# adr-arroyo/PointCloudComparator

Hardware: AMD Instinct MI355X
Metric: nn_queries_per_sec (higher is better)
Workload: dtype f32; 1 GPU; C3: 10M x 10M XYZRGB (32-B stride), k=1 NN; step = index build over 10000000 references + 10000000 queries on each GPU (10000000 over 1 GPU); backend=none, engine=grid, references=10000000, queries_per_gpu=10000000, queries_total=10000000, point_stride_bytes=32

## Files before the change

### pointcloudcomparator_amd/csrc/cellsort_mp.hip

```cpp
#include "pcc_internal.hpp"
#include "grid_device.hpp"
#include "lane_ops.hpp"
#include <algorithm>

namespace pcc {

constexpr int MP_T = 256;
constexpr unsigned int MP_F2 = 2048;
constexpr unsigned int MP_B2 = 128;
constexpr unsigned int MP_MAX_B1 = 256;
constexpr unsigned int MP_MAX_G = 512;
constexpr unsigned int MP_SLICE2 = 8192;
constexpr unsigned int MP_STAGE_BYTES = 32768;
constexpr unsigned int MP_WIN = 8;
#ifndef PCC_MP_STAGE_PTS
#define PCC_MP_STAGE_PTS 3072
#endif
#ifndef PCC_MP_STAGE_ORD
#define PCC_MP_STAGE_ORD 6144
#endif
constexpr unsigned int MP_FINE_STAGE_PTS = PCC_MP_STAGE_PTS, MP_FINE_STAGE_ORD = PCC_MP_STAGE_ORD;

struct MpPlan {
    unsigned int F1, F2, B1, G1, slice1;
};
static MpPlan mp_plan(unsigned int ncells_cap, unsigned int n) {
    MpPlan p;
    p.F2 = MP_F2;
    while ((unsigned long long)p.F2 * MP_B2 * MP_MAX_B1 < (unsigned long long)ncells_cap + 1) p.F2 *= 2;
    p.F1 = p.F2 * MP_B2;
    p.B1 = (ncells_cap + p.F1) / p.F1;
    p.G1 = (n + 16383) / 16384;
    if (p.G1 > MP_MAX_G) p.G1 = MP_MAX_G;
    if (p.G1 < 1) p.G1 = 1;
    p.slice1 = (n + p.G1 - 1) / p.G1;
    return p;
}

__device__ __forceinline__ unsigned int mp_cell(const float4& v, const GridParams& g, bool voxel) {
    return voxel ? voxel_id(v, g) : cell_id(v, g);
}
__device__ __forceinline__ unsigned int mp_cell(const uint2& v, const GridParams&, bool) { return v.x; }
__device__ __forceinline__ unsigned int mp_position(const float4& v) { return (unsigned int)__float_as_int(v.w); }
__device__ __forceinline__ unsigned int mp_position(const uint2& v) { return v.y; }
template <class E> __device__ __forceinline__ E mp_make(const float4& v, unsigned int cell, unsigned int pos);
template <> __device__ __forceinline__ float4 mp_make<float4>(const float4& v, unsigned int, unsigned int) { return v; }
template <> __device__ __forceinline__ uint2 mp_make<uint2>(const float4&, unsigned int cell, unsigned int pos) { return make_uint2(cell, pos); }

__global__ void __launch_bounds__(MP_T)
k_mp_hist1(const float4* __restrict__ pts, unsigned int n, const GridDev* __restrict__ gd, unsigned int F1, unsigned int B1,
           unsigned int slice, unsigned int* __restrict__ H, unsigned int* __restrict__ zero, unsigned int n_zero) {
    for (unsigned int z = blockIdx.x * MP_T + threadIdx.x; z < n_zero; z += gridDim.x * MP_T) zero[z] = 0u;
    __shared__ unsigned int cnt[MP_MAX_B1];
    const GridParams g = gd->g;
    const bool voxel = gd->voxel != 0;
    for (unsigned int b = threadIdx.x; b < B1; b += MP_T) cnt[b] = 0;
    __syncthreads();
    const unsigned int beg = blockIdx.x * slice, end = min(n, beg + slice);
    for (unsigned int i0 = beg + threadIdx.x; i0 < end; i0 += 4 * MP_T) {
        float4 v[4];
#pragma unroll
        for (int u = 0; u < 4; ++u)
            if (i0 + u * MP_T < end) v[u] = pts[i0 + u * MP_T];
#pragma unroll
        for (int u = 0; u < 4; ++u)
            if (i0 + u * MP_T < end && __float_as_int(v[u].w) >= 0) atomicAdd(&cnt[mp_cell(v[u], g, voxel) / F1], 1u);
    }
    __syncthreads();
    for (unsigned int b = threadIdx.x; b < B1; b += MP_T) H[(size_t)b * gridDim.x + blockIdx.x] = cnt[b];
    if (blockIdx.x == 0 && threadIdx.x == 0) H[(size_t)B1 * gridDim.x] = 0;
}

template <class E>
__global__ void __launch_bounds__(MP_T)
k_mp_scatter1(const float4* __restrict__ pts, unsigned int n, const GridDev* __restrict__ gd, unsigned int F1, unsigned int B1,
              unsigned int slice, const unsigned int* __restrict__ H, E* __restrict__ out) {
    __shared__ unsigned int cur[MP_MAX_B1];
    const GridParams g = gd->g;
    const bool voxel = gd->voxel != 0;
    for (unsigned int b = threadIdx.x; b < B1; b += MP_T) cur[b] = H[(size_t)b * gridDim.x + blockIdx.x];
    __syncthreads();
    const unsigned int beg = blockIdx.x * slice, end = min(n, beg + slice);
    for (unsigned int i0 = beg + threadIdx.x; i0 < end; i0 += 4 * MP_T) {
        float4 v[4];
#pragma unroll
        for (int u = 0; u < 4; ++u)
            if (i0 + u * MP_T < end) v[u] = pts[i0 + u * MP_T];
#pragma unroll
        for (int u = 0; u < 4; ++u)
            if (i0 + u * MP_T < end && __float_as_int(v[u].w) >= 0) {
                const unsigned int c = mp_cell(v[u], g, voxel);
                out[atomicAdd(&cur[c / F1], 1u)] = mp_make<E>(v[u], c, i0 + u * MP_T);
            }
    }
}

__global__ void __launch_bounds__(MP_T)
k_mp_hist1_cells(const unsigned int* __restrict__ cells, unsigned int n, unsigned int F1, unsigned int B1, unsigned int slice,
                 unsigned int* __restrict__ H, unsigned int* __restrict__ zero, unsigned int n_zero) {
    for (unsigned int z = blockIdx.x * MP_T + threadIdx.x; z < n_zero; z += gridDim.x * MP_T) zero[z] = 0u;
    __shared__ unsigned int cnt[MP_MAX_B1];
    for (unsigned int b = threadIdx.x; b < B1; b += MP_T) cnt[b] = 0;
    __syncthreads();
    const unsigned int beg = blockIdx.x * slice, end = min(n, beg + slice);
    for (unsigned int i0 = beg + threadIdx.x; i0 < end; i0 += 8 * MP_T) {
        unsigned int c[8];
#pragma unroll
        for (int u = 0; u < 8; ++u) c[u] = i0 + u * MP_T < end ? cells[i0 + u * MP_T] : 0xffffffffu;
#pragma unroll
        for (int u = 0; u < 8; ++u)
            if (c[u] != 0xffffffffu) atomicAdd(&cnt[c[u] / F1], 1u);
    }
    __syncthreads();
    for (unsigned int b = threadIdx.x; b < B1; b += MP_T) H[(size_t)b * gridDim.x + blockIdx.x] = cnt[b];
    if (blockIdx.x == 0 && threadIdx.x == 0) H[(size_t)B1 * gridDim.x] = 0;
}
__global__ void __launch_bounds__(MP_T)
k_mp_scatter1_cells(const unsigned int* __restrict__ cells, unsigned int n, unsigned int F1, unsigned int B1, unsigned int slice,
                    const unsigned int* __restrict__ H, uint2* __restrict__ out) {
    __shared__ unsigned int cur[MP_MAX_B1];
    for (unsigned int b = threadIdx.x; b < B1; b += MP_T) cur[b] = H[(size_t)b * gridDim.x + blockIdx.x];
    __syncthreads();
    const unsigned int beg = blockIdx.x * slice, end = min(n, beg + slice);
    for (unsigned int i0 = beg + threadIdx.x; i0 < end; i0 += 8 * MP_T) {
        unsigned int c[8];
#pragma unroll
        for (int u = 0; u < 8; ++u) c[u] = i0 + u * MP_T < end ? cells[i0 + u * MP_T] : 0xffffffffu;
#pragma unroll
        for (int u = 0; u < 8; ++u)
            if (c[u] != 0xffffffffu) out[atomicAdd(&cur[c[u] / F1], 1u)] = make_uint2(c[u], i0 + u * MP_T);
    }
}

constexpr unsigned int MP_TILE1 = 2048;
template <class E>
__global__ void __launch_bounds__(MP_T)
k_mp_scatter1_staged(const float4* __restrict__ pts, unsigned int n, const GridDev* __restrict__ gd, unsigned int F1, unsigned int B1,
                     unsigned int slice, const unsigned int* __restrict__ H, E* __restrict__ out) {
    constexpr int PER = MP_TILE1 / MP_T;
    __shared__ unsigned int cur[MP_MAX_B1], tcnt[MP_MAX_B1], tstart[MP_MAX_B1];
    __shared__ unsigned short sb[MP_TILE1];
    __shared__ __attribute__((aligned(16))) unsigned char stage_raw[MP_TILE1 * sizeof(E)];
    E* stage = reinterpret_cast<E*>(stage_raw);
    const GridParams g = gd->g;
    const bool voxel = gd->voxel != 0;
    for (unsigned int b = threadIdx.x; b < B1; b += MP_T) cur[b] = H[(size_t)b * gridDim.x + blockIdx.x];
    const unsigned int beg = blockIdx.x * slice, end = min(n, beg + slice);
    for (unsigned int t0 = beg; t0 < end; t0 += MP_TILE1) {
        for (unsigned int b = threadIdx.x; b < MP_MAX_B1; b += MP_T) tcnt[b] = 0;
        __syncthreads();
        float4 v[PER];
        unsigned int bk[PER], rk[PER];
#pragma unroll
        for (int u = 0; u < PER; ++u) {
            const unsigned int i = t0 + threadIdx.x + u * MP_T;
            v[u] = make_float4(0.f, 0.f, 0.f, __int_as_float(-1));
            if (i < end) v[u] = pts[i];
        }
#pragma unroll
        for (int u = 0; u < PER; ++u) {
            bk[u] = 0xffffffffu;
            rk[u] = 0;
            if (__float_as_int(v[u].w) >= 0) {
                bk[u] = mp_cell(v[u], g, voxel);
                rk[u] = atomicAdd(&tcnt[bk[u] / F1], 1u);
            }
        }
        __syncthreads();
        if (threadIdx.x < 64) {
            unsigned int c[4], sum = 0;
#pragma unroll
            for (int j = 0; j < 4; ++j) { c[j] = tcnt[4 * threadIdx.x + j]; sum += c[j]; }
            unsigned int ex = wave_incl_scan_add(sum) - sum;
#pragma unroll
            for (int j = 0; j < 4; ++j) { tstart[4 * threadIdx.x + j] = ex; ex += c[j]; }
        }
        __syncthreads();
#pragma unroll
        for (int u = 0; u < PER; ++u)
            if (bk[u] != 0xffffffffu) {
                const unsigned int b = bk[u] / F1, slot = tstart[b] + rk[u];
                stage[slot] = mp_make<E>(v[u], bk[u], t0 + threadIdx.x + u * MP_T);
                sb[slot] = (unsigned short)b;
            }
        __syncthreads();
        const unsigned int tile_n = tstart[MP_MAX_B1 - 1] + tcnt[MP_MAX_B1 - 1];
        for (unsigned int j = threadIdx.x; j < tile_n; j += MP_T) {
            const unsigned int b = sb[j];
            out[cur[b] + (j - tstart[b])] = stage[j];
        }
        __syncthreads();
        for (unsigned int b = threadIdx.x; b < MP_MAX_B1; b += MP_T) cur[b] += tcnt[b];
    }
}

__device__ __forceinline__ unsigned int mp_pair(unsigned int c, unsigned int F1, unsigned int F2) {
    return (c / F1) * MP_B2 + (c % F1) / F2;
}

template <bool PLACE, class E>
__global__ void __launch_bounds__(MP_T)
k_mp_level2(const E* __restrict__ in, const unsigned int* __restrict__ n_valid_ptr, const GridDev* __restrict__ gd,
            unsigned int F1, unsigned int F2, unsigned int* __restrict__ C, E* __restrict__ out) {
    constexpr unsigned int SLICE = PLACE ? MP_STAGE_BYTES / sizeof(E) : MP_SLICE2;
    __shared__ unsigned int cnt[MP_WIN * MP_B2];
    __shared__ __attribute__((aligned(16))) unsigned char stage_raw[PLACE ? MP_STAGE_BYTES : 16];
    E* stage = reinterpret_cast<E*>(stage_raw);
    const GridParams g = gd->g;
    const bool voxel = gd->voxel != 0;
    const unsigned int n = *n_valid_ptr;
    const unsigned int beg = blockIdx.x * SLICE, end = min(n, beg + SLICE);
    if (beg >= end) return;
    const unsigned int w0 = (mp_cell(in[beg], g, voxel) / F1) * MP_B2;
    for (unsigned int k = threadIdx.x; k < MP_WIN * MP_B2; k += MP_T) cnt[k] = 0;
    __syncthreads();
    for (unsigned int i0 = beg + threadIdx.x; i0 < end; i0 += 4 * MP_T) {
        E v[4];
#pragma unroll
        for (int u = 0; u < 4; ++u)
            if (i0 + u * MP_T < end) v[u] = in[i0 + u * MP_T];
#pragma unroll
        for (int u = 0; u < 4; ++u) {
            if (i0 + u * MP_T >= end) break;
            if (PLACE) stage[i0 + u * MP_T - beg] = v[u];
            const unsigned int pr = mp_pair(mp_cell(v[u], g, voxel), F1, F2);
            if (pr - w0 < MP_WIN * MP_B2) atomicAdd(&cnt[pr - w0], 1u);
            else if (!PLACE) atomicAdd(&C[pr], 1u);
            else out[atomicAdd(&C[pr], 1u)] = v[u];
        }
    }
    __syncthreads();
    for (unsigned int k = threadIdx.x; k < MP_WIN * MP_B2; k += MP_T) {
        const unsigned int c = cnt[k];
        if (c) {
            if (!PLACE) atomicAdd(&C[w0 + k], c);
            else cnt[k] = atomicAdd(&C[w0 + k], c);
        }
    }
    if (!PLACE) return;
    __syncthreads();
    for (unsigned int j = threadIdx.x; j < end - beg; j += MP_T) {
        const E v = stage[j];
        const unsigned int pr = mp_pair(mp_cell(v, g, voxel), F1, F2);
        if (pr - w0 < MP_WIN * MP_B2) out[atomicAdd(&cnt[pr - w0], 1u)] = v;
    }
}

__device__ __forceinline__ void mp_store_point(float4* out, unsigned int pos, const float4& v) { if (out) out[pos] = v; }
__device__ __forceinline__ void mp_store_point(float4*, unsigned int, const uint2&) {}

template <bool REFS, class E>
__device__ __forceinline__ void mp_fine_block(unsigned int* lds, const E* __restrict__ in, unsigned int beg, unsigned int end, unsigned int cell0,
                                              const GridParams& g, bool voxel, unsigned int F2, float4* __restrict__ out_pts,
                                              unsigned int* __restrict__ out_order, unsigned int* __restrict__ cell_start) {
    unsigned int* cnt = lds;
    unsigned int* wsum = lds + F2;
    const unsigned int ncells = (unsigned int)g.ncells;
    for (unsigned int f = threadIdx.x; f < F2; f += MP_T) cnt[f] = 0;
    __syncthreads();
    for (unsigned int j0 = beg + threadIdx.x; j0 < end; j0 += 4 * MP_T) {
        E v[4];
#pragma unroll
        for (int u = 0; u < 4; ++u)
            if (j0 + u * MP_T < end) v[u] = in[j0 + u * MP_T];
#pragma unroll
        for (int u = 0; u < 4; ++u)
            if (j0 + u * MP_T < end) atomicAdd(&cnt[mp_cell(v[u], g, voxel) - cell0], 1u);
    }
    __syncthreads();
    const unsigned int per = (F2 + MP_T - 1) / MP_T;
    const unsigned int f0 = threadIdx.x * per, f1 = min(F2, f0 + per);
    unsigned int s = 0;
    for (unsigned int f = f0; f < f1; ++f) s += cnt[f];
    const unsigned int lane = threadIdx.x & 63, wave = threadIdx.x >> 6;
    const unsigned int inc = wave_incl_scan_add(s);
    if (lane == 63) wsum[wave] = inc;
    __syncthreads();
    unsigned int run = beg + inc - s;
    for (unsigned int w = 0; w < wave; ++w) run += wsum[w];
    for (unsigned int f = f0; f < f1; ++f) {
        const unsigned int c = cnt[f];
        cnt[f] = run;
        if (REFS && cell0 + f <= ncells) cell_start[cell0 + f] = run;
        run += c;
    }
    __syncthreads();
    const unsigned int stage_cap = out_pts ? MP_FINE_STAGE_PTS : MP_FINE_STAGE_ORD;
    const bool staged = end - beg <= stage_cap;
    float4* st_pts = reinterpret_cast<float4*>(lds + ((F2 + 4 + 3) & ~3u));
    unsigned int* st_ord = reinterpret_cast<unsigned int*>(st_pts + (out_pts ? MP_FINE_STAGE_PTS : 0));
    for (unsigned int j0 = beg + threadIdx.x; j0 < end; j0 += 4 * MP_T) {
        E v[4];
#pragma unroll
        for (int u = 0; u < 4; ++u)
            if (j0 + u * MP_T < end) v[u] = in[j0 + u * MP_T];
#pragma unroll
        for (int u = 0; u < 4; ++u) {
            if (j0 + u * MP_T >= end) break;
            const unsigned int pos = atomicAdd(&cnt[mp_cell(v[u], g, voxel) - cell0], 1u);
            if (staged) {
                mp_store_point(out_pts ? st_pts : nullptr, pos - beg, v[u]);
                if (out_order) st_ord[pos - beg] = mp_position(v[u]);
            } else {
                mp_store_point(out_pts, pos, v[u]);
                if (out_order) out_order[pos] = mp_position(v[u]);
            }
        }
    }
    if (staged) {
        __syncthreads();
        for (unsigned int i = threadIdx.x; i < end - beg; i += MP_T) {
            if (out_pts) out_pts[beg + i] = st_pts[i];
            if (out_order) out_order[beg + i] = st_ord[i];
        }
    }
}

#ifndef PCC_MP_LIGHT_PTS
#define PCC_MP_LIGHT_PTS 1024
#endif
#ifndef PCC_MP_LIGHT_ORD
#define PCC_MP_LIGHT_ORD 1024
#endif
template <class E> struct MpWave;
template <> struct MpWave<float4> {
    typedef float4 Staged;
    static constexpr unsigned int LIGHT = PCC_MP_LIGHT_PTS;
    static __device__ __forceinline__ float4 staged(const float4& v) { return v; }
    static __device__ __forceinline__ void store(float4* out_pts, unsigned int*, unsigned int pos, const float4& v) { out_pts[pos] = v; }
};
template <> struct MpWave<uint2> {
    typedef unsigned int Staged;
    static constexpr unsigned int LIGHT = PCC_MP_LIGHT_ORD;
    static __device__ __forceinline__ unsigned int staged(const uint2& v) { return v.y; }
    static __device__ __forceinline__ void store(float4*, unsigned int* out_order, unsigned int pos, unsigned int v) { out_order[pos] = v; }
};
template <class E> constexpr unsigned int mp_wave_words() {
    return MP_F2 / 2 + MpWave<E>::LIGHT * (unsigned int)(sizeof(typename MpWave<E>::Staged) / sizeof(unsigned int));
}
static_assert(PCC_MP_LIGHT_PTS % 64 == 0 && PCC_MP_LIGHT_ORD % 64 == 0 && PCC_MP_LIGHT_PTS < 65536 && PCC_MP_LIGHT_ORD < 65536,
              "a light bucket is whole rounds of a wave and fits a 16-bit counter");

template <bool REFS, class E>
__device__ __forceinline__ void mp_fine_wave(unsigned int* cnt , const E* __restrict__ in, unsigned int beg, unsigned int n,
                                             unsigned int cell0, const GridParams& g, bool voxel, float4* __restrict__ out_pts,
                                             unsigned int* __restrict__ out_order, unsigned int* __restrict__ cell_start) {
    typedef MpWave<E> W;
    constexpr unsigned int PER = W::LIGHT / 64;
    const unsigned int ncells = (unsigned int)g.ncells;
    const unsigned int lane = threadIdx.x & 63;
    if (n == 0) {
        for (unsigned int f = lane; f < MP_F2; f += 64)
            if (cell0 + f <= ncells) cell_start[cell0 + f] = beg;
        return;
    }
    unsigned short* cnt16 = reinterpret_cast<unsigned short*>(cnt);
    typename W::Staged* stage = reinterpret_cast<typename W::Staged*>(cnt + MP_F2 / 2);
    E v[PER];
#pragma unroll
    for (unsigned int u = 0; u < PER; ++u) v[u] = in[beg + min(lane + 64 * u, n - 1)];
    for (unsigned int k = lane; k < MP_F2 / 8; k += 64) reinterpret_cast<uint4*>(cnt)[k] = make_uint4(0u, 0u, 0u, 0u);
    wave_lds_sync();
    unsigned int key[PER];
#pragma unroll
    for (unsigned int u = 0; u < PER; ++u)
        if (lane + 64 * u < n) {
            const unsigned int c = (mp_cell(v[u], g, voxel) - cell0) & (MP_F2 - 1), sh = 16 * (c & 1);
            const unsigned int old = atomicAdd(&cnt[c >> 1], 1u << sh);
            key[u] = c | ((old >> sh) & 0xffffu) << 16;
        }
    wave_lds_sync();
    unsigned int base = 0;
#pragma unroll 8
    for (unsigned int step = 0; step < MP_F2 / 64; ++step) {
        const unsigned int f = 64 * step + lane;
        const unsigned int c = cnt16[f];
        const unsigned int inc = wave_incl_scan_add(c);
        const unsigned int first = base + inc - c;
        cnt16[f] = (unsigned short)first;
        if (REFS && cell0 + f <= ncells) cell_start[cell0 + f] = beg + first;
        base += __builtin_amdgcn_readlane(inc, 63);
    }
    wave_lds_sync();
#pragma unroll
    for (unsigned int u = 0; u < PER; ++u)
        if (lane + 64 * u < n) key[u] = cnt16[key[u] & 0xffffu] + (key[u] >> 16);
#pragma unroll
    for (unsigned int u = 0; u < PER; ++u)
        if (lane + 64 * u < n) stage[key[u]] = W::staged(v[u]);
    wave_lds_sync();
    for (unsigned int i = lane; i < n; i += 64) W::store(out_pts, out_order, beg + i, stage[i]);
}

template <class E> constexpr unsigned int mp_once_cap() { return MP_T * MpWave<E>::LIGHT / 64; }
template <class E> constexpr unsigned int mp_once_words() {
    return MP_F2 + 4 + mp_once_cap<E>() * (unsigned int)(sizeof(typename MpWave<E>::Staged) / sizeof(unsigned int));
}
template <bool REFS, class E>
__device__ __forceinline__ void mp_fine_once(unsigned int* lds, const E* __restrict__ in, unsigned int beg, unsigned int n, unsigned int cell0,
                                             const GridParams& g, bool voxel, float4* __restrict__ out_pts,
                                             unsigned int* __restrict__ out_order, unsigned int* __restrict__ cell_start) {
    typedef MpWave<E> W;
    constexpr unsigned int PER = W::LIGHT / 64;
    unsigned int* cnt = lds;
    unsigned int* wsum = lds + MP_F2;
    typename W::Staged* stage = reinterpret_cast<typename W::Staged*>(lds + MP_F2 + 4);
    const unsigned int ncells = (unsigned int)g.ncells;
    E v[PER];
#pragma unroll
    for (unsigned int u = 0; u < PER; ++u) v[u] = in[beg + min(threadIdx.x + MP_T * u, n - 1)];
    for (unsigned int f = threadIdx.x; f < MP_F2; f += MP_T) cnt[f] = 0;
    __syncthreads();
    unsigned int key[PER];
#pragma unroll
    for (unsigned int u = 0; u < PER; ++u)
        if (threadIdx.x + MP_T * u < n) {
            const unsigned int c = (mp_cell(v[u], g, voxel) - cell0) & (MP_F2 - 1);
            key[u] = c | atomicAdd(&cnt[c], 1u) << 16;
        }
    __syncthreads();
    constexpr unsigned int per = MP_F2 / MP_T;
    const unsigned int f0 = threadIdx.x * per;
    unsigned int s = 0;
#pragma unroll
    for (unsigned int f = f0; f < f0 + per; ++f) s += cnt[f];
    const unsigned int lane = threadIdx.x & 63, wave = threadIdx.x >> 6;
    const unsigned int inc = wave_incl_scan_add(s);
    if (lane == 63) wsum[wave] = inc;
    __syncthreads();
    unsigned int run = inc - s;
    for (unsigned int w = 0; w < wave; ++w) run += wsum[w];
#pragma unroll
    for (unsigned int f = f0; f < f0 + per; ++f) {
        const unsigned int c = cnt[f];
        cnt[f] = run;
        if (REFS && cell0 + f <= ncells) cell_start[cell0 + f] = beg + run;
        run += c;
    }
    __syncthreads();
#pragma unroll
    for (unsigned int u = 0; u < PER; ++u)
        if (threadIdx.x + MP_T * u < n) key[u] = cnt[key[u] & 0xffffu] + (key[u] >> 16);
#pragma unroll
    for (unsigned int u = 0; u < PER; ++u)
        if (threadIdx.x + MP_T * u < n) stage[key[u]] = W::staged(v[u]);
    __syncthreads();
    for (unsigned int i = threadIdx.x; i < n; i += MP_T) W::store(out_pts, out_order, beg + i, stage[i]);
}
static_assert(MP_T * PCC_MP_LIGHT_PTS / 64 < 65536 && MP_T * PCC_MP_LIGHT_ORD / 64 < 65536, "a rank of the one-read block form fits 16 bits");

template <bool REFS, class E>
__global__ void __launch_bounds__(MP_T)
k_mp_fine(const E* __restrict__ in, const unsigned int* __restrict__ ends , const GridDev* __restrict__ gd,
          unsigned int F2, unsigned int n_block, unsigned int light, float4* __restrict__ out_pts, unsigned int* __restrict__ out_order,
          unsigned int* __restrict__ cell_start) {
    extern __shared__ __attribute__((aligned(16))) unsigned int lds[];
    const GridParams g = gd->g;
    const bool voxel = gd->voxel != 0;
    const unsigned int ncells = (unsigned int)g.ncells;
    const bool block = blockIdx.x < n_block;
    const unsigned int wave = __builtin_amdgcn_readfirstlane(threadIdx.x >> 6);
    const unsigned int b = block ? blockIdx.x : 4 * (blockIdx.x - n_block) + wave;
    const unsigned int cell0 = b * F2;
    if (cell0 > ncells) return;
    const unsigned int beg = b ? ends[b - 1] : 0u, end = ends[b];
    if (!REFS && beg == end) return;
    if (block) {
        if (light == 0 || end - beg > mp_once_cap<E>()) mp_fine_block<REFS, E>(lds, in, beg, end, cell0, g, voxel, F2, out_pts, out_order, cell_start);
        else if (end - beg > light) mp_fine_once<REFS, E>(lds, in, beg, end - beg, cell0, g, voxel, out_pts, out_order, cell_start);
    } else if (end - beg <= light) {
        mp_fine_wave<REFS, E>(lds + wave * mp_wave_words<E>(), in, beg, end - beg, cell0, g, voxel, out_pts, out_order, cell_start);
    }
}

int cell_sort_mp(pcc_index* ix, const float4* pts, size_t n_pts, bool refs, float4* out_pts, unsigned int* out_order,
                 unsigned int* cell_start, unsigned int** n_sorted_dev, const GridDev* gd_override,
                 unsigned int nc_cap_override) {
    hipStream_t s = ix->stream;
    const unsigned int n = (unsigned int)n_pts;
    const unsigned int ncap = gd_override ? nc_cap_override : ix->nc_cap;
    const MpPlan p = mp_plan(ncap, n);
    const GridDev* gd = gd_override ? gd_override : ix->d_grid.as<GridDev>();
    const unsigned int np = p.B1 * MP_B2;
    PCC_TRY(ix->mp_a.reserve((size_t)n * sizeof(float4) + 256));
    PCC_TRY(ix->mp_b.reserve((size_t)n * sizeof(float4) + 256));
    const size_t h_elems = (size_t)p.B1 * p.G1 + 1;
    PCC_TRY(ix->scratch_b.reserve(((h_elems + 3) & ~(size_t)3) * sizeof(unsigned int)));
    PCC_TRY(ix->mp_c.reserve(((size_t)np + 8) * sizeof(unsigned int)));
    unsigned int* H = ix->scratch_b.as<unsigned int>();
    unsigned int* C = ix->mp_c.as<unsigned int>();
    const unsigned int* cells = nullptr;
    if (!refs && !out_pts && !gd_override && pts == ix->q_packed.as<float4>() && ix->q_cells_n == n_pts && n_pts != 0)
        cells = ix->q_cells.as<unsigned int>();
    if (!refs) ix->q_cells_n = 0;
    if (cells)
        hipLaunchKernelGGL(k_mp_hist1_cells, dim3(p.G1), dim3(MP_T), 0, s, cells, n, p.F1, p.B1, p.slice1, H, C, np);
    else
    hipLaunchKernelGGL(k_mp_hist1, dim3(p.G1), dim3(MP_T), 0, s, pts, n, gd, p.F1, p.B1, p.slice1, H, C, np);
    PCC_HIP(hipGetLastError());
    PCC_TRY(launch_exclusive_scan(ix, s, H, h_elems, ix->scratch_a));
    unsigned int* n_valid = H + h_elems - 1;
    if (n_sorted_dev) *n_sorted_dev = n_valid;
    const size_t lds3_block = (((size_t)p.F2 + 4 + 3) & ~(size_t)3) * sizeof(unsigned int) +
                              (out_pts ? (size_t)MP_FINE_STAGE_PTS * (sizeof(float4) + (out_order ? sizeof(unsigned int) : 0))
                                       : (size_t)MP_FINE_STAGE_ORD * sizeof(unsigned int));
    const unsigned int light = p.F2 != MP_F2 || (out_pts != nullptr) == (out_order != nullptr) ? 0u : out_pts ? MpWave<float4>::LIGHT : MpWave<uint2>::LIGHT;
    const size_t lds3_wave = !light ? 0 : 4 * sizeof(unsigned int) * (out_pts ? mp_wave_words<float4>() : mp_wave_words<uint2>());
    const size_t lds3_once = !light ? 0 : sizeof(unsigned int) * (out_pts ? mp_once_words<float4>() : mp_once_words<uint2>());
    const size_t lds3 = std::max(lds3_block, std::max(lds3_wave, lds3_once));
    const unsigned int g3 = np + (light ? np / 4 : 0u);
    const unsigned int g2c = (n + MP_SLICE2 - 1) / MP_SLICE2;
    if (out_pts) {
        float4* t1 = ix->mp_a.as<float4>();
        float4* t2 = ix->mp_b.as<float4>();
        const unsigned int g2p = (n + MP_STAGE_BYTES / sizeof(float4) - 1) / (MP_STAGE_BYTES / sizeof(float4));
        if (ix->opt.sort_stage1)
            hipLaunchKernelGGL((k_mp_scatter1_staged<float4>), dim3(p.G1), dim3(MP_T), 0, s, pts, n, gd, p.F1, p.B1, p.slice1, H, t1);
        else
            hipLaunchKernelGGL((k_mp_scatter1<float4>), dim3(p.G1), dim3(MP_T), 0, s, pts, n, gd, p.F1, p.B1, p.slice1, H, t1);
        hipLaunchKernelGGL((k_mp_level2<false, float4>), dim3(g2c), dim3(MP_T), 0, s, t1, n_valid, gd, p.F1, p.F2, C, t2);
        PCC_TRY(launch_exclusive_scan(ix, s, C, np, ix->scratch_a));
        hipLaunchKernelGGL((k_mp_level2<true, float4>), dim3(g2p), dim3(MP_T), 0, s, t1, n_valid, gd, p.F1, p.F2, C, t2);
        if (refs)
            hipLaunchKernelGGL((k_mp_fine<true, float4>), dim3(g3), dim3(MP_T), lds3, s, t2, C, gd, p.F2, np, light, out_pts, out_order, cell_start);
        else
            hipLaunchKernelGGL((k_mp_fine<false, float4>), dim3(g3), dim3(MP_T), lds3, s, t2, C, gd, p.F2, np, light, out_pts, out_order, cell_start);
    } else {
        uint2* t1 = ix->mp_a.as<uint2>();
        uint2* t2 = ix->mp_b.as<uint2>();
        const unsigned int g2p = (n + MP_STAGE_BYTES / sizeof(uint2) - 1) / (MP_STAGE_BYTES / sizeof(uint2));
        if (cells)
            hipLaunchKernelGGL(k_mp_scatter1_cells, dim3(p.G1), dim3(MP_T), 0, s, cells, n, p.F1, p.B1, p.slice1, H, t1);
        else if (ix->opt.sort_stage1 == 2)
            hipLaunchKernelGGL((k_mp_scatter1_staged<uint2>), dim3(p.G1), dim3(MP_T), 0, s, pts, n, gd, p.F1, p.B1, p.slice1, H, t1);
        else
            hipLaunchKernelGGL((k_mp_scatter1<uint2>), dim3(p.G1), dim3(MP_T), 0, s, pts, n, gd, p.F1, p.B1, p.slice1, H, t1);
        hipLaunchKernelGGL((k_mp_level2<false, uint2>), dim3(g2c), dim3(MP_T), 0, s, t1, n_valid, gd, p.F1, p.F2, C, t2);
        PCC_TRY(launch_exclusive_scan(ix, s, C, np, ix->scratch_a));
        hipLaunchKernelGGL((k_mp_level2<true, uint2>), dim3(g2p), dim3(MP_T), 0, s, t1, n_valid, gd, p.F1, p.F2, C, t2);
        if (refs)
            hipLaunchKernelGGL((k_mp_fine<true, uint2>), dim3(g3), dim3(MP_T), lds3, s, t2, C, gd, p.F2, np, light, out_pts, out_order, cell_start);
        else
            hipLaunchKernelGGL((k_mp_fine<false, uint2>), dim3(g3), dim3(MP_T), lds3, s, t2, C, gd, p.F2, np, light, out_pts, out_order, cell_start);
    }
    PCC_HIP(hipGetLastError());
    return PCC_OK;
}

}
```

Baseline: 7.041 billion queries/s.

## Persist level-2 placement blocks with LDS-sorted staging and add heavy-bucket fine kernel

The level-2 placement kernel becomes persistent: a capped grid walks several slices per block and prefetches the next slice while the current one is written. Each slice is locally counting-sorted in LDS, so in-window points go out as contiguous coalesced runs instead of scattered per-point atomics. Mid-sized fine buckets for the float4 path are listed by a new kernel and sorted by 1024-thread blocks with large LDS staging, and the regular fine kernel skips those buckets. The cost is more launches, a hipFuncSetAttribute call on every sort, extra scratch for the list, and more LDS and barriers per block.

```diff
diff --git a/pointcloudcomparator_amd/csrc/cellsort_mp.hip b/pointcloudcomparator_amd/csrc/cellsort_mp.hip
--- a/pointcloudcomparator_amd/csrc/cellsort_mp.hip
+++ b/pointcloudcomparator_amd/csrc/cellsort_mp.hip
@@ -198,52 +198,130 @@
     return (c / F1) * MP_B2 + (c % F1) / F2;
 }
 
+#ifndef PCC_MP_L2_WGS
+#define PCC_MP_L2_WGS 1024
+#endif
+#ifndef PCC_MP_L2_WGS_ORD
+#define PCC_MP_L2_WGS_ORD 1536
+#endif
+static_assert(MP_WIN * MP_B2 <= 65536 && MP_STAGE_BYTES / sizeof(uint2) <= 65536 && (MP_WIN * MP_B2) % MP_T == 0 && PCC_MP_L2_WGS > 0 && PCC_MP_L2_WGS_ORD > 0,
+              "a window slot and a rank inside a slice fit 16 bits each; a thread owns whole counters");
+
 template <bool PLACE, class E>
 __global__ void __launch_bounds__(MP_T)
 k_mp_level2(const E* __restrict__ in, const unsigned int* __restrict__ n_valid_ptr, const GridDev* __restrict__ gd,
-            unsigned int F1, unsigned int F2, unsigned int* __restrict__ C, E* __restrict__ out) {
+            unsigned int F1, unsigned int F2, unsigned int* __restrict__ C, E* __restrict__ out, unsigned int slices) {
     constexpr unsigned int SLICE = PLACE ? MP_STAGE_BYTES / sizeof(E) : MP_SLICE2;
-    __shared__ unsigned int cnt[MP_WIN * MP_B2];
+    constexpr unsigned int NWIN = MP_WIN * MP_B2;
+    __shared__ unsigned int cnt[NWIN];
     __shared__ __attribute__((aligned(16))) unsigned char stage_raw[PLACE ? MP_STAGE_BYTES : 16];
-    E* stage = reinterpret_cast<E*>(stage_raw);
+    __shared__ __attribute__((aligned(16))) unsigned short sb[PLACE ? SLICE : 16];
     const GridParams g = gd->g;
     const bool voxel = gd->voxel != 0;
     const unsigned int n = *n_valid_ptr;
-    const unsigned int beg = blockIdx.x * SLICE, end = min(n, beg + SLICE);
-    if (beg >= end) return;
-    const unsigned int w0 = (mp_cell(in[beg], g, voxel) / F1) * MP_B2;
-    for (unsigned int k = threadIdx.x; k < MP_WIN * MP_B2; k += MP_T) cnt[k] = 0;
-    __syncthreads();
-    for (unsigned int i0 = beg + threadIdx.x; i0 < end; i0 += 4 * MP_T) {
-        E v[4];
-#pragma unroll
-        for (int u = 0; u < 4; ++u)
-            if (i0 + u * MP_T < end) v[u] = in[i0 + u * MP_T];
-#pragma unroll
-        for (int u = 0; u < 4; ++u) {
-            if (i0 + u * MP_T >= end) break;
-            if (PLACE) stage[i0 + u * MP_T - beg] = v[u];
-            const unsigned int pr = mp_pair(mp_cell(v[u], g, voxel), F1, F2);
-            if (pr - w0 < MP_WIN * MP_B2) atomicAdd(&cnt[pr - w0], 1u);
-            else if (!PLACE) atomicAdd(&C[pr], 1u);
-            else out[atomicAdd(&C[pr], 1u)] = v[u];
-        }
-    }
-    __syncthreads();
-    for (unsigned int k = threadIdx.x; k < MP_WIN * MP_B2; k += MP_T) {
-        const unsigned int c = cnt[k];
-        if (c) {
-            if (!PLACE) atomicAdd(&C[w0 + k], c);
-            else cnt[k] = atomicAdd(&C[w0 + k], c);
-        }
-    }
-    if (!PLACE) return;
-    __syncthreads();
-    for (unsigned int j = threadIdx.x; j < end - beg; j += MP_T) {
-        const E v = stage[j];
-        const unsigned int pr = mp_pair(mp_cell(v, g, voxel), F1, F2);
-        if (pr - w0 < MP_WIN * MP_B2) out[atomicAdd(&cnt[pr - w0], 1u)] = v;
-    }
+    if constexpr (PLACE) {
+        constexpr unsigned int PER = SLICE / MP_T, OWN = NWIN / MP_T;
+        E* stage = reinterpret_cast<E*>(stage_raw);
+        unsigned int* wsum = reinterpret_cast<unsigned int*>(sb);
+        unsigned int* w0s = reinterpret_cast<unsigned int*>(sb) + 4;
+        unsigned int beg = (unsigned int)((unsigned long long)blockIdx.x * slices / gridDim.x) * SLICE;
+        const unsigned int stop = (unsigned int)min((unsigned long long)n, (unsigned long long)(blockIdx.x + 1) * slices / gridDim.x * SLICE);
+        if (beg >= stop) return;
+        E v[PER];
+#pragma unroll
+        for (unsigned int u = 0; u < PER; ++u) v[u] = in[min(beg + threadIdx.x + u * MP_T, beg + min(stop - beg, SLICE) - 1)];
+        for (;;) {
+            const unsigned int end = beg + min(stop - beg, SLICE), nbeg = beg + SLICE;
+            const bool more = stop - beg > SLICE;
+            if (threadIdx.x == 0) *w0s = (mp_cell(v[0], g, voxel) / F1) * MP_B2;
+            for (unsigned int k = threadIdx.x; k < NWIN; k += MP_T) cnt[k] = 0;
+            __syncthreads();
+            const unsigned int w0 = *w0s;
+            unsigned int key[PER];
+#pragma unroll
+            for (unsigned int u = 0; u < PER; ++u) {
+                key[u] = 0xffffffffu;
+                if (beg + threadIdx.x + u * MP_T < end) {
+                    const unsigned int pr = mp_pair(mp_cell(v[u], g, voxel), F1, F2);
+                    if (pr - w0 < NWIN) key[u] = (pr - w0) | atomicAdd(&cnt[pr - w0], 1u) << 16;
+                    else out[atomicAdd(&C[pr], 1u)] = v[u];
+                }
+            }
+            __syncthreads();
+            unsigned int c[OWN], s = 0;
+#pragma unroll
+            for (unsigned int j = 0; j < OWN; ++j) { c[j] = cnt[OWN * threadIdx.x + j]; s += c[j]; }
+            const unsigned int inc = wave_incl_scan_add(s);
+            if ((threadIdx.x & 63) == 63) wsum[threadIdx.x >> 6] = inc;
+            __syncthreads();
+            unsigned int first = inc - s, staged = 0;
+#pragma unroll
+            for (unsigned int w = 0; w < MP_T / 64; ++w) {
+                if (w < (threadIdx.x >> 6)) first += wsum[w];
+                staged += wsum[w];
+            }
+            unsigned int delta[OWN];
+#pragma unroll
+            for (unsigned int j = 0; j < OWN; ++j) {
+                cnt[OWN * threadIdx.x + j] = first;
+                delta[j] = c[j] ? atomicAdd(&C[w0 + OWN * threadIdx.x + j], c[j]) - first : 0u;
+                first += c[j];
+            }
+            __syncthreads();
+            unsigned int slot[PER];
+#pragma unroll
+            for (unsigned int u = 0; u < PER; ++u)
+                slot[u] = key[u] != 0xffffffffu ? cnt[key[u] & 0xffffu] + (key[u] >> 16) : 0u;
+#pragma unroll
+            for (unsigned int u = 0; u < PER; ++u)
+                if (key[u] != 0xffffffffu) {
+                    stage[slot[u]] = v[u];
+                    sb[slot[u]] = (unsigned short)key[u];
+                }
+            if (more) {
+#pragma unroll
+                for (unsigned int u = 0; u < PER; ++u) v[u] = in[min(nbeg + threadIdx.x + u * MP_T, nbeg + min(stop - nbeg, SLICE) - 1)];
+            }
+            __syncthreads();
+#pragma unroll
+            for (unsigned int j = 0; j < OWN; ++j) cnt[OWN * threadIdx.x + j] = delta[j];
+            __syncthreads();
+            for (unsigned int j = threadIdx.x; j < staged; j += MP_T) out[cnt[sb[j]] + j] = stage[j];
+            if (!more) return;
+            __syncthreads();
+            beg = nbeg;
+        }
+    } else {
+        const unsigned int beg = blockIdx.x * SLICE, end = min(n, beg + SLICE);
+        if (beg >= end) return;
+        const unsigned int w0 = (mp_cell(in[beg], g, voxel) / F1) * MP_B2;
+        for (unsigned int k = threadIdx.x; k < NWIN; k += MP_T) cnt[k] = 0;
+        __syncthreads();
+        for (unsigned int i0 = beg + threadIdx.x; i0 < end; i0 += 4 * MP_T) {
+            E v[4];
+#pragma unroll
+            for (int u = 0; u < 4; ++u)
+                if (i0 + u * MP_T < end) v[u] = in[i0 + u * MP_T];
+#pragma unroll
+            for (int u = 0; u < 4; ++u) {
+                if (i0 + u * MP_T >= end) break;
+                const unsigned int pr = mp_pair(mp_cell(v[u], g, voxel), F1, F2);
+                if (pr - w0 < NWIN) atomicAdd(&cnt[pr - w0], 1u);
+                else atomicAdd(&C[pr], 1u);
+            }
+        }
+        __syncthreads();
+        for (unsigned int k = threadIdx.x; k < NWIN; k += MP_T) {
+            const unsigned int c = cnt[k];
+            if (c) atomicAdd(&C[w0 + k], c);
+        }
+    }
+}
+
+template <class E> static void mp_place2_grid(unsigned int n, unsigned int* slices, unsigned int* grid) {
+    const unsigned int slice = MP_STAGE_BYTES / (unsigned int)sizeof(E);
+    *slices = (n + slice - 1) / slice;
+    *grid = std::min(*slices, (unsigned int)(sizeof(E) == sizeof(float4) ? PCC_MP_L2_WGS : PCC_MP_L2_WGS_ORD));
 }
 
 __device__ __forceinline__ void mp_store_point(float4* out, unsigned int pos, const float4& v) { if (out) out[pos] = v; }
@@ -452,8 +530,8 @@
 template <bool REFS, class E>
 __global__ void __launch_bounds__(MP_T)
 k_mp_fine(const E* __restrict__ in, const unsigned int* __restrict__ ends , const GridDev* __restrict__ gd,
-          unsigned int F2, unsigned int n_block, unsigned int light, float4* __restrict__ out_pts, unsigned int* __restrict__ out_order,
-          unsigned int* __restrict__ cell_start) {
+          unsigned int F2, unsigned int n_block, unsigned int light, unsigned int heavy, float4* __restrict__ out_pts,
+          unsigned int* __restrict__ out_order, unsigned int* __restrict__ cell_start) {
     extern __shared__ __attribute__((aligned(16))) unsigned int lds[];
     const GridParams g = gd->g;
     const bool voxel = gd->voxel != 0;
@@ -466,11 +544,93 @@
     const unsigned int beg = b ? ends[b - 1] : 0u, end = ends[b];
     if (!REFS && beg == end) return;
     if (block) {
+        if (end - beg > mp_once_cap<E>() && end - beg <= heavy) return;
         if (light == 0 || end - beg > mp_once_cap<E>()) mp_fine_block<REFS, E>(lds, in, beg, end, cell0, g, voxel, F2, out_pts, out_order, cell_start);
         else if (end - beg > light) mp_fine_once<REFS, E>(lds, in, beg, end - beg, cell0, g, voxel, out_pts, out_order, cell_start);
     } else if (end - beg <= light) {
         mp_fine_wave<REFS, E>(lds + wave * mp_wave_words<E>(), in, beg, end - beg, cell0, g, voxel, out_pts, out_order, cell_start);
     }
+}
+
+#ifndef PCC_MP_HEAVY_PTS
+#define PCC_MP_HEAVY_PTS 12288
+#endif
+constexpr int MP_TH = 1024;
+constexpr unsigned int MP_HEAVY_STAGE = 9216;
+constexpr unsigned int MP_HEAVY_WGS = 256;
+constexpr unsigned int mp_heavy_words() { return MP_F2 + 16 + MP_HEAVY_STAGE * 4; }
+static_assert(PCC_MP_HEAVY_PTS % MP_TH == 0 && PCC_MP_HEAVY_PTS < 65536 && mp_heavy_words() * 4 <= 160 * 1024, "a rank fits 16 bits; the stage fits LDS");
+__global__ void __launch_bounds__(MP_T)
+k_mp_heavy_list(const unsigned int* __restrict__ ends, unsigned int np, unsigned int lo, unsigned int* __restrict__ count, unsigned int* __restrict__ list) {
+    const unsigned int b = blockIdx.x * MP_T + threadIdx.x;
+    if (b >= np) return;
+    const unsigned int n = ends[b] - (b ? ends[b - 1] : 0u);
+    if (n > lo && n <= PCC_MP_HEAVY_PTS) list[atomicAdd(count, 1u)] = b;
+}
+template <bool REFS>
+__global__ void __launch_bounds__(MP_TH)
+k_mp_fine_heavy(const float4* __restrict__ in, const unsigned int* __restrict__ ends, const GridDev* __restrict__ gd,
+                const unsigned int* __restrict__ count, const unsigned int* __restrict__ list, float4* __restrict__ out_pts,
+                unsigned int* __restrict__ cell_start) {
+    extern __shared__ __attribute__((aligned(16))) unsigned int lds[];
+    constexpr unsigned int PER = PCC_MP_HEAVY_PTS / MP_TH, per = MP_F2 / MP_TH;
+    const GridParams g = gd->g;
+    const bool voxel = gd->voxel != 0;
+    const unsigned int total = *count;
+  for (unsigned int j = blockIdx.x; j < total; j += gridDim.x) {
+    const unsigned int b = list[j];
+    const unsigned int beg = b ? ends[b - 1] : 0u, n = ends[b] - beg;
+    const unsigned int ncells = (unsigned int)g.ncells, cell0 = b * MP_F2;
+    unsigned int* cnt = lds;
+    unsigned int* wsum = lds + MP_F2;
+    float4* stage = reinterpret_cast<float4*>(lds + MP_F2 + 16);
+    float4 v[PER];
+#pragma unroll
+    for (unsigned int u = 0; u < PER; ++u) v[u] = in[beg + min(threadIdx.x + MP_TH * u, n - 1)];
+    for (unsigned int f = threadIdx.x; f < MP_F2; f += MP_TH) cnt[f] = 0;
+    __syncthreads();
+    unsigned int key[PER];
+#pragma unroll
+    for (unsigned int u = 0; u < PER; ++u)
+        if (threadIdx.x + MP_TH * u < n) {
+            const unsigned int c = (mp_cell(v[u], g, voxel) - cell0) & (MP_F2 - 1);
+            key[u] = c | atomicAdd(&cnt[c], 1u) << 16;
+        }
+    __syncthreads();
+    const unsigned int f0 = threadIdx.x * per;
+    unsigned int s = 0;
+#pragma unroll
+    for (unsigned int f = f0; f < f0 + per; ++f) s += cnt[f];
+    const unsigned int lane = threadIdx.x & 63, wave = threadIdx.x >> 6;
+    const unsigned int inc = wave_incl_scan_add(s);
+    if (lane == 63) wsum[wave] = inc;
+    __syncthreads();
+    unsigned int run = inc - s;
+    for (unsigned int w = 0; w < wave; ++w) run += wsum[w];
+#pragma unroll
+    for (unsigned int f = f0; f < f0 + per; ++f) {
+        const unsigned int c = cnt[f];
+        cnt[f] = run;
+        if (REFS && cell0 + f <= ncells) cell_start[cell0 + f] = beg + run;
+        run += c;
+    }
+    __syncthreads();
+#pragma unroll
+    for (unsigned int u = 0; u < PER; ++u)
+        if (threadIdx.x + MP_TH * u < n) key[u] = cnt[key[u] & 0xffffu] + (key[u] >> 16);
+    if (n <= MP_HEAVY_STAGE) {
+#pragma unroll
+        for (unsigned int u = 0; u < PER; ++u)
+            if (threadIdx.x + MP_TH * u < n) stage[key[u]] = v[u];
+        __syncthreads();
+        for (unsigned int i = threadIdx.x; i < n; i += MP_TH) out_pts[beg + i] = stage[i];
+    } else {
+#pragma unroll
+        for (unsigned int u = 0; u < PER; ++u)
+            if (threadIdx.x + MP_TH * u < n) out_pts[beg + key[u]] = v[u];
+    }
+    __syncthreads();
+  }
 }
 
 int cell_sort_mp(pcc_index* ix, const float4* pts, size_t n_pts, bool refs, float4* out_pts, unsigned int* out_order,
@@ -486,7 +646,7 @@
     PCC_TRY(ix->mp_b.reserve((size_t)n * sizeof(float4) + 256));
     const size_t h_elems = (size_t)p.B1 * p.G1 + 1;
     PCC_TRY(ix->scratch_b.reserve(((h_elems + 3) & ~(size_t)3) * sizeof(unsigned int)));
-    PCC_TRY(ix->mp_c.reserve(((size_t)np + 8) * sizeof(unsigned int)));
+    PCC_TRY(ix->mp_c.reserve((2 * (size_t)np + 16) * sizeof(unsigned int)));
     unsigned int* H = ix->scratch_b.as<unsigned int>();
     unsigned int* C = ix->mp_c.as<unsigned int>();
     const unsigned int* cells = nullptr;
@@ -494,9 +654,9 @@
         cells = ix->q_cells.as<unsigned int>();
     if (!refs) ix->q_cells_n = 0;
     if (cells)
-        hipLaunchKernelGGL(k_mp_hist1_cells, dim3(p.G1), dim3(MP_T), 0, s, cells, n, p.F1, p.B1, p.slice1, H, C, np);
+        hipLaunchKernelGGL(k_mp_hist1_cells, dim3(p.G1), dim3(MP_T), 0, s, cells, n, p.F1, p.B1, p.slice1, H, C, np + 8);
     else
-    hipLaunchKernelGGL(k_mp_hist1, dim3(p.G1), dim3(MP_T), 0, s, pts, n, gd, p.F1, p.B1, p.slice1, H, C, np);
+    hipLaunchKernelGGL(k_mp_hist1, dim3(p.G1), dim3(MP_T), 0, s, pts, n, gd, p.F1, p.B1, p.slice1, H, C, np + 8);
     PCC_HIP(hipGetLastError());
     PCC_TRY(launch_exclusive_scan(ix, s, H, h_elems, ix->scratch_a));
     unsigned int* n_valid = H + h_elems - 1;
@@ -509,39 +669,51 @@
     const size_t lds3_once = !light ? 0 : sizeof(unsigned int) * (out_pts ? mp_once_words<float4>() : mp_once_words<uint2>());
     const size_t lds3 = std::max(lds3_block, std::max(lds3_wave, lds3_once));
     const unsigned int g3 = np + (light ? np / 4 : 0u);
+    const unsigned int heavy = light && out_pts ? PCC_MP_HEAVY_PTS : 0u;
     const unsigned int g2c = (n + MP_SLICE2 - 1) / MP_SLICE2;
     if (out_pts) {
         float4* t1 = ix->mp_a.as<float4>();
         float4* t2 = ix->mp_b.as<float4>();
-        const unsigned int g2p = (n + MP_STAGE_BYTES / sizeof(float4) - 1) / (MP_STAGE_BYTES / sizeof(float4));
+        unsigned int sl2, g2p;
+        mp_place2_grid<float4>(n, &sl2, &g2p);
         if (ix->opt.sort_stage1)
             hipLaunchKernelGGL((k_mp_scatter1_staged<float4>), dim3(p.G1), dim3(MP_T), 0, s, pts, n, gd, p.F1, p.B1, p.slice1, H, t1);
         else
             hipLaunchKernelGGL((k_mp_scatter1<float4>), dim3(p.G1), dim3(MP_T), 0, s, pts, n, gd, p.F1, p.B1, p.slice1, H, t1);
-        hipLaunchKernelGGL((k_mp_level2<false, float4>), dim3(g2c), dim3(MP_T), 0, s, t1, n_valid, gd, p.F1, p.F2, C, t2);
+        hipLaunchKernelGGL((k_mp_level2<false, float4>), dim3(g2c), dim3(MP_T), 0, s, t1, n_valid, gd, p.F1, p.F2, C, t2, 0u);
         PCC_TRY(launch_exclusive_scan(ix, s, C, np, ix->scratch_a));
-        hipLaunchKernelGGL((k_mp_level2<true, float4>), dim3(g2p), dim3(MP_T), 0, s, t1, n_valid, gd, p.F1, p.F2, C, t2);
+        hipLaunchKernelGGL((k_mp_level2<true, float4>), dim3(g2p), dim3(MP_T), 0, s, t1, n_valid, gd, p.F1, p.F2, C, t2, sl2);
+        if (heavy) {
+            const size_t ldsh = mp_heavy_words() * sizeof(unsigned int);
+            PCC_HIP(hipFuncSetAttribute(refs ? (const void*)k_mp_fine_heavy<true> : (const void*)k_mp_fine_heavy<false>, hipFuncAttributeMaxDynamicSharedMemorySize, (int)ldsh));
+            unsigned int* h_count = C + np + 4;
+            unsigned int* h_list = C + np + 8;
+            hipLaunchKernelGGL(k_mp_heavy_list, dim3((np + MP_T - 1) / MP_T), dim3(MP_T), 0, s, C, np, mp_once_cap<float4>(), h_count, h_list);
+            if (refs) hipLaunchKernelGGL((k_mp_fine_heavy<true>), dim3(MP_HEAVY_WGS), dim3(MP_TH), ldsh, s, t2, C, gd, h_count, h_list, out_pts, cell_start);
+            else hipLaunchKernelGGL((k_mp_fine_heavy<false>), dim3(MP_HEAVY_WGS), dim3(MP_TH), ldsh, s, t2, C, gd, h_count, h_list, out_pts, cell_start);
+        }
         if (refs)
-            hipLaunchKernelGGL((k_mp_fine<true, float4>), dim3(g3), dim3(MP_T), lds3, s, t2, C, gd, p.F2, np, light, out_pts, out_order, cell_start);
+            hipLaunchKernelGGL((k_mp_fine<true, float4>), dim3(g3), dim3(MP_T), lds3, s, t2, C, gd, p.F2, np, light, heavy, out_pts, out_order, cell_start);
         else
-            hipLaunchKernelGGL((k_mp_fine<false, float4>), dim3(g3), dim3(MP_T), lds3, s, t2, C, gd, p.F2, np, light, out_pts, out_order, cell_start);
+            hipLaunchKernelGGL((k_mp_fine<false, float4>), dim3(g3), dim3(MP_T), lds3, s, t2, C, gd, p.F2, np, light, heavy, out_pts, out_order, cell_start);
     } else {
         uint2* t1 = ix->mp_a.as<uint2>();
         uint2* t2 = ix->mp_b.as<uint2>();
-        const unsigned int g2p = (n + MP_STAGE_BYTES / sizeof(uint2) - 1) / (MP_STAGE_BYTES / sizeof(uint2));
+        unsigned int sl2, g2p;
+        mp_place2_grid<uint2>(n, &sl2, &g2p);
         if (cells)
             hipLaunchKernelGGL(k_mp_scatter1_cells, dim3(p.G1), dim3(MP_T), 0, s, cells, n, p.F1, p.B1, p.slice1, H, t1);
         else if (ix->opt.sort_stage1 == 2)
             hipLaunchKernelGGL((k_mp_scatter1_staged<uint2>), dim3(p.G1), dim3(MP_T), 0, s, pts, n, gd, p.F1, p.B1, p.slice1, H, t1);
         else
             hipLaunchKernelGGL((k_mp_scatter1<uint2>), dim3(p.G1), dim3(MP_T), 0, s, pts, n, gd, p.F1, p.B1, p.slice1, H, t1);
-        hipLaunchKernelGGL((k_mp_level2<false, uint2>), dim3(g2c), dim3(MP_T), 0, s, t1, n_valid, gd, p.F1, p.F2, C, t2);
+        hipLaunchKernelGGL((k_mp_level2<false, uint2>), dim3(g2c), dim3(MP_T), 0, s, t1, n_valid, gd, p.F1, p.F2, C, t2, 0u);
         PCC_TRY(launch_exclusive_scan(ix, s, C, np, ix->scratch_a));
-        hipLaunchKernelGGL((k_mp_level2<true, uint2>), dim3(g2p), dim3(MP_T), 0, s, t1, n_valid, gd, p.F1, p.F2, C, t2);
+        hipLaunchKernelGGL((k_mp_level2<true, uint2>), dim3(g2p), dim3(MP_T), 0, s, t1, n_valid, gd, p.F1, p.F2, C, t2, sl2);
         if (refs)
-            hipLaunchKernelGGL((k_mp_fine<true, uint2>), dim3(g3), dim3(MP_T), lds3, s, t2, C, gd, p.F2, np, light, out_pts, out_order, cell_start);
+            hipLaunchKernelGGL((k_mp_fine<true, uint2>), dim3(g3), dim3(MP_T), lds3, s, t2, C, gd, p.F2, np, light, heavy, out_pts, out_order, cell_start);
         else
-            hipLaunchKernelGGL((k_mp_fine<false, uint2>), dim3(g3), dim3(MP_T), lds3, s, t2, C, gd, p.F2, np, light, out_pts, out_order, cell_start);
+            hipLaunchKernelGGL((k_mp_fine<false, uint2>), dim3(g3), dim3(MP_T), lds3, s, t2, C, gd, p.F2, np, light, heavy, out_pts, out_order, cell_start);
     }
     PCC_HIP(hipGetLastError());
     return PCC_OK;
```

Result: faster. 7.231 billion queries/s (median of 6 runs) (+2.7%).
